# maxdoblas/QuickEd

Measured on AMD Instinct MI355X. Metric: alignments/sec + GCUPS, 10kb x 10kb 5%-error pairs, higher is better.
Workload: dtype u64; 1 GPU; banded_score, DEVICE-RESIDENT inputs: 100000 pairs/GPU x 10000 bp @ 0.05 error, bandwidth 15 %, seeded generator (SURVEY 8d), ASCII already in HBM when the clock starts, results left in HBM (end-to-end rates: e2e); pairs_per_gpu=100000, length=10000, bandwidth=15, parallelism=pairs sharded over 1 GPU(s), no data-path collective

## Files before the change

quicked_amd/csrc/qe_kernels.hip:

```cpp
#include <type_traits>
#include <hip/hip_runtime.h>
#include "qe_types.h"
#include "qe_bounded.h"
#include "qe_search.h"
#include "qe_panel.h"
#include "qe_panel_align.h"
#include "qe_pack.h"
#include "qe_tags.h"
#include "qe_check.h"

namespace qe {

#define QE_ONES (~(u64)0)
#define QE_WAVE_IN_BLOCK() ((int)(threadIdx.x >> 6))
#define QE_GROUP_INDEX() ((int)(blockIdx.x * (blockDim.x >> 6) + (threadIdx.x >> 6)))
extern __shared__ uint4 qe_dyn_lds[];

__device__ __forceinline__ u32 lo32(u64 x) { return (u32)x; }
__device__ __forceinline__ u32 hi32(u64 x) { return (u32)(x >> 32); }
__device__ __forceinline__ u64 mk64(u32 lo, u32 hi) { return ((u64)hi << 32) | lo; }

__device__ __forceinline__ int64_t tile_elem(int col, int slot, int nslots) {
    return ((int64_t)(col >> 3) * nslots + slot) * 512 + (col & 7);
}
// ... 317 lines not shown

template <int K>
__device__ __forceinline__ void run64_tall(u64 (&P)[K], u64 (&M)[K], const u64 (&a)[K], const u64 (&b)[K],
                                           u64 T0, u64 T1, u64 hinP, u64 hinM, u64& houtP, u64& houtM) {
    u32 alo[K], ahi[K], blo[K], bhi[K], Plo[K], Phi[K], Mlo[K], Mhi[K];
#pragma unroll
    for (int k = 0; k < K; ++k) {
        alo[k] = lo32(a[k]); ahi[k] = hi32(a[k]); blo[k] = lo32(b[k]); bhi[k] = hi32(b[k]);
        Plo[k] = lo32(P[k]); Phi[k] = hi32(P[k]); Mlo[k] = lo32(M[k]); Mhi[k] = hi32(M[k]);
    }
    u32 oPlo = 0, oPhi = 0, oMlo = 0, oMhi = 0;
#pragma unroll 1
    for (int half = 0; half < 2; ++half) {
        const u32 t0 = half ? hi32(T0) : lo32(T0), t1 = half ? hi32(T1) : lo32(T1);
        const u32 hp = half ? hi32(hinP) : lo32(hinP), hm = half ? hi32(hinM) : lo32(hinM);
        u32 gP = 0, gM = 0;
#pragma unroll 1
        for (int c = 0; c < 32; c += 2) {
            u32 m0[2], m1[2], cP[2], cM[2];
#pragma unroll
            for (int j = 0; j < 2; ++j) {
                m0[j] = (u32)__builtin_amdgcn_sbfe((int)t0, (u32)(c + j), 1u);
                m1[j] = (u32)__builtin_amdgcn_sbfe((int)t1, (u32)(c + j), 1u);
                cP[j] = __builtin_amdgcn_ubfe(hp, (u32)(c + j), 1u);
                cM[j] = __builtin_amdgcn_ubfe(hm, (u32)(c + j), 1u);
            }
#pragma unroll
            for (int s = 0; s <= K; ++s) {
#pragma unroll
                for (int j = 0; j < 2; ++j) {
                    const int k = s - j;
                    if (k < 0 || k >= K) continue;
                    const u32 elo = bitop3<0x90>(~(alo[k] ^ m0[j]), blo[k], m1[j]), ehi = bitop3<0x90>(~(ahi[k] ^ m0[j]), bhi[k], m1[j]);
                    if (k + 1 < K) {
                        u32 phhi, mhhi;
                        block_step_core(elo, ehi, Plo[k], Phi[k], Mlo[k], Mhi[k], cP[j], cM[j], phhi, mhhi);
                        cP[j] = phhi >> 31; cM[j] = mhhi >> 31;
                    } else {
                        block_step_collect(elo, ehi, Plo[k], Phi[k], Mlo[k], Mhi[k], cP[j], cM[j], gP, gM);
                    }
                }
            }
        }
        const u32 rP = __builtin_bitreverse32(gP), rM = __builtin_bitreverse32(gM);
        if (half) { oPhi = rP; oMhi = rM; } else { oPlo = rP; oMlo = rM; }
    }
#pragma unroll
    for (int k = 0; k < K; ++k) { P[k] = mk64(Plo[k], Phi[k]); M[k] = mk64(Mlo[k], Mhi[k]); }
    houtP = mk64(oPlo, oPhi);
    houtM = mk64(oMlo, oMhi);
}

template <int K>
__device__ __forceinline__ void slots_pass_tall(int nl, int i, int r, u64* Pv, u64* Mv, int32_t* S, const u64* pp, int p0, bool unaligned,
                                                u64 T0, u64 T1, u64& hinP, u64& hinM, u32& adv) {
    u64 P[K], M[K], a[K], b[K], a1[K], b1[K];
    int sc[K], v0[K];
    const int psh = p0 & 63;
#pragma unroll
    for (int k = 0; k < K; ++k) {
        P[k] = 0; M[k] = 0; a[k] = 0; b[k] = 0; a1[k] = 0; b1[k] = 0; sc[k] = 0;
        if (k < nl) {
            P[k] = Pv[(int64_t)(i + k) * 64]; M[k] = Mv[(int64_t)(i + k) * 64]; sc[k] = S[(int64_t)score_lds_row(r + k) * 64];
            const u64* w = pp + 3 * (int64_t)((p0 >> 6) + r + k);
            a[k] = w[0]; b[k] = w[1];
            if (unaligned) { a1[k] = w[3]; b1[k] = w[4]; }
        }
    }
    if (unaligned) {
#pragma unroll
        for (int k = 0; k < K; ++k) {
            a[k] = (a[k] >> psh) | ((a1[k] << 1) << (63 - psh));
            b[k] = (b[k] >> psh) | ((b1[k] << 1) << (63 - psh));
        }
    }
#pragma unroll
    for (int k = 0; k < K; ++k) v0[k] = __popcll(P[k]) - __popcll(M[k]);
    u64 houtP, houtM;
    run64_tall<K>(P, M, a, b, T0, T1, hinP, hinM, houtP, houtM);
    if (nl > 0) {
        int d = __popcll(houtP) - __popcll(houtM);
#pragma unroll
        for (int k = K - 1; k >= 0; --k) {
            if (k < nl) {
                S[(int64_t)score_lds_row(r + k) * 64] = sc[k] + d;
                Pv[(int64_t)(i + k - 1) * 64] = P[k]; Mv[(int64_t)(i + k - 1) * 64] = M[k];
            }
            d -= (__popcll(P[k]) - __popcll(M[k])) - v0[k];
        }
        adv += 64u * (u32)nl;
    }
    hinP = houtP; hinM = houtM;
}

__device__ __forceinline__ void run64_win2(u64& P0, u64& M0, u64& P1, u64& M1, u64 a0, u64 b0, u64 a1, u64 b1, u64 T0, u64 T1,
                                           u64 hinP, bool patch, u64 Eq_x, u64& gP, u64& gM, uint4* st, int st_stride) {
    const u32 a0lo = lo32(a0), a0hi = hi32(a0), b0lo = lo32(b0), b0hi = hi32(b0);
    const u32 a1lo = lo32(a1), a1hi = hi32(a1), b1lo = lo32(b1), b1hi = hi32(b1);
    u32 P0lo = lo32(P0), P0hi = hi32(P0), M0lo = lo32(M0), M0hi = hi32(M0);
    u32 P1lo = lo32(P1), P1hi = hi32(P1), M1lo = lo32(M1), M1hi = hi32(M1);
    u32 oPlo = 0, oPhi = 0, oMlo = 0, oMhi = 0;
#pragma unroll 1
    for (int half = 0; half < 2; ++half) {
        const u32 t0 = half ? hi32(T0) : lo32(T0), t1 = half ? hi32(T1) : lo32(T1);
        const u32 hp = half ? hi32(hinP) : lo32(hinP);
        u32 g0P = 0, g0M = 0;
        u32 m0[32], m1[32];
#pragma unroll
        for (int s = 0; s < 33; ++s) {
            if (s < 32) {
                m0[s] = (u32)__builtin_amdgcn_sbfe((int)t0, s, 1);
                m1[s] = (u32)__builtin_amdgcn_sbfe((int)t1, s, 1);
            }
            if (s >= 1) {
                const int c = s - 1;
                if ((c & 7) == 0) st[(4 * half + (c >> 3)) * st_stride] = make_uint4(P1lo, P1hi, M1lo, M1hi);
                u32 inP = g0P & 1u, inM = g0M & 1u;
                if (c == 31 && half == 1 && patch) {
                    u64 Ph, Mh, Pe = mk64(P0lo, P0hi), Me = mk64(M0lo, M0hi);
                    block_step(Eq_x, Pe, Me, 1u, 0u, Ph, Mh);
                    inP = (u32)(Ph >> 63); inM = (u32)(Mh >> 63);
                    g0P = (g0P & ~1u) | inP; g0M = (g0M & ~1u) | inM;
                }
                const u32 elo = bitop3<0x90>(~(a1lo ^ m0[c]), b1lo, m1[c]), ehi = bitop3<0x90>(~(a1hi ^ m0[c]), b1hi, m1[c]);
                u32 ph_, mh_;
                block_step_core(elo, ehi, P1lo, P1hi, M1lo, M1hi, inP, inM, ph_, mh_);
            }
            if (s < 32) {
                const u32 elo = bitop3<0x90>(~(a0lo ^ m0[s]), b0lo, m1[s]), ehi = bitop3<0x90>(~(a0hi ^ m0[s]), b0hi, m1[s]);
                block_step_fused(elo, ehi, P0lo, P0hi, M0lo, M0hi, __builtin_amdgcn_ubfe(hp, s, 1), 0u, g0P, g0M);
            }
        }
        const u32 rP = __builtin_bitreverse32(g0P), rM = __builtin_bitreverse32(g0M);
        if (half) { oPhi = rP; oMhi = rM; } else { oPlo = rP; oMlo = rM; }
    }
    P0 = mk64(P0lo, P0hi); M0 = mk64(M0lo, M0hi); P1 = mk64(P1lo, P1hi); M1 = mk64(M1lo, M1hi);
    gP = mk64(oPlo, oPhi); gM = mk64(oMlo, oMhi);
}
// ... 390 lines not shown

__global__ __launch_bounds__(256) void k_planes_iupac(IupacPlanesArgs A) {
    const int lane = threadIdx.x & 63;
    const int seq = blockIdx.x * 4 + (threadIdx.x >> 6);
    if (seq >= A.nseq) return;
    const int len = A.len[seq];
    const int nw = (len + 63) >> 6;
    const u64* __restrict__ src = A.src + A.pl_off[seq];
    u64* __restrict__ dst = A.dst + iupac_offset(A.pl_off[seq]);
    for (int r = lane; r < nw + 2; r += 64) {
        u64 o[4] = {0, 0, 0, 0};
        if (r < nw) iupac_row_from_planes3(src[3 * (int64_t)r], src[3 * (int64_t)r + 1], src[3 * (int64_t)r + 2], min(len - 64 * r, 64), A.n_empty != 0, o);
        u64* q = dst + 4 * (int64_t)r;
        q[0] = o[0]; q[1] = o[1]; q[2] = o[2]; q[3] = o[3];
    }
}

struct Geom { int cutoff, diff, prolog, ebb, fin; };
__device__ __forceinline__ Geom band_geometry(int m, int n, int cutoff_in) {
    Geom g;
    const int kend = abs(n - m) + 1;
    g.cutoff = max(max(kend, cutoff_in), 65);
    g.diff = m - n;
    const int rel = (g.cutoff - abs(g.diff) + 1) / 2;
    if (g.diff >= 0) {
        g.prolog = (rel + 63) / 64;
        g.ebb = (rel + g.diff + 63) / 64 + 1 + g.prolog;
    } else {
        g.prolog = (rel - g.diff + 63) / 64;
        g.ebb = (rel + 63) / 64 + 1 + g.prolog;
    }
    g.fin = g.prolog * 64 + g.diff;
    return g;
}

struct GroupWs {
    u64* Pv; u64* Mv; int32_t* S; int16_t* cf; int16_t* cl;
};
__device__ __forceinline__ GroupWs group_ws(uint8_t* ws, int64_t off, int ns, int nrows, int nch) {
    GroupWs w;
    uint8_t* p = ws + off;
    w.Pv = (u64*)p;              p += (int64_t)(ns + 1) * 64 * 8;
    w.Mv = (u64*)p;              p += (int64_t)(ns + 1) * 64 * 8;
    w.S = (int32_t*)p;           p += (int64_t)nrows * 64 * 4;
    w.cf = (int16_t*)p;          p += (int64_t)nch * 64 * 2;
    w.cl = (int16_t*)p;
    return w;
}

#ifndef QE_FILL_K
#define QE_FILL_K 3
#endif
constexpr bool QE_K_BANDED_LDS = true;
template <bool FILL, bool LDS = false>
__global__ __launch_bounds__(512) void k_banded(BandedArgs A) {
    static_assert(!(FILL && LDS), "the fill's state stays in the group workspace");
    const int g = QE_GROUP_INDEX(), lane = threadIdx.x & 63, t = g * 64 + lane;
    if (g * 64 >= A.T.ntasks) return;
    int pair = (t < A.T.ntasks) ? A.T.pair[t] : -1;
    if (A.only_if != nullptr && pair >= 0 && A.only_if[t] == 0) pair = -1;
    const bool have = pair >= 0;
    if (!__any(have)) return;
    int m = 1, n = 1, p0 = 0, t0 = 0, cut_in = 0, tfin = 0, prune = 0x7fffffff;
    const u64* pp = A.P.pl_p;
    const u64* tp = A.P.pl_t;
    u32 fl = 0;
    if (have) {
        m = A.T.m[t]; n = A.T.n[t]; p0 = A.T.p0[t]; t0 = A.T.t0[t];
        cut_in = A.T.cutoff[t];
        tfin = FILL ? n : A.T.tfin[t];
        if (!FILL && A.prune != nullptr) prune = A.prune[t];
        pp = A.P.pl_p + A.P.pl_p_off[pair];
        tp = A.P.pl_t + A.P.pl_t_off[pair];
        fl = A.P.flags[pair];
    }
    const bool hasN = (fl & FLAG_HAS_N) != 0;
    const Geom G = band_geometry(m, n, cut_in);
    const int thr = prune < cut_in ? prune : G.cutoff;
    const int nw = (m + 63) >> 6;
    const bool fgeom = FILL || (!LDS && A.fill_geom != 0);
    const int nsl = fgeom ? G.ebb : ((G.cutoff + 63) >> 6) + 1;
    const int stop_row = fgeom ? nw - 1 : nw;
    const int lvl_last = (m - 1) & 63;
    int first = G.prolog, last = nsl - 1, pos_v = -G.prolog, pos_h = 0;
    int max_row_init = nsl - 1;
    u32 adv = 0;

    const int gns = LDS ? A.lds_slots : A.g_nslots[g], gnr = LDS ? 0 : A.g_nrows[g], gnch = LDS ? 0 : A.g_nch[g];
    GroupWs W;
    if (LDS) {
        uint8_t* lb = (uint8_t*)qe_dyn_lds + (size_t)QE_WAVE_IN_BLOCK() * (size_t)score_lds_bytes(gns);
        W.Pv = (u64*)lb; W.Mv = W.Pv + (gns + 1) * 64; W.S = (int32_t*)(W.Mv + (gns + 1) * 64); W.cf = nullptr; W.cl = nullptr;
        if (nsl > gns) pair = -1;
    } else W = group_ws(A.ws, A.g_ws_off[g], gns, gnr, gnch);
    const bool valid = pair >= 0;
    u64* const Pv = W.Pv + 64 + lane;
    u64* const Mv = W.Mv + 64 + lane;
    int32_t* const S = W.S + lane;
    auto srow = [](int r) { return (int64_t)(LDS ? score_lds_row(r) : r) * 64; };
    uint4* const cp = FILL ? A.mat + A.g_mat_off[g] + lane : nullptr;
    const int64_t cps = (int64_t)gns * 64;
    uint4* const hw = FILL ? cp + (int64_t)QE_CPC * gnch * cps : nullptr;

    for (int s = 0; s < gns; ++s) {
        if (valid && s < nsl) {
            Pv[(int64_t)s * 64] = QE_ONES;
            Mv[(int64_t)s * 64] = 0;
            S[srow(s)] = 64 * (s + 1);
            if (FILL) cp[(int64_t)s * 64] = make_uint4(~0u, ~0u, 0u, 0u);
        }
    }
    if (FILL && valid) { W.cf[lane] = (int16_t)first; W.cl[lane] = (int16_t)last; }

    const int nfull = tfin >> 6, tail = tfin & 63;
    const int my_chunks = valid ? nfull + (tail ? 1 : 0) : 0;
    const int wave_chunks = wave_max(my_chunks);

    for (int k = 0; k < wave_chunks; ++k) {
        const int ncols = (k < nfull) ? 64 : ((k == nfull) ? tail : 0);
        const bool on = valid && ncols > 0;
        u64 T0 = 0, T1 = 0, TN = 0;
        if (on) load_planes(tp, t0 + 64 * k, T0, T1, TN);
        const int rhi = min(last, nw - 1 - pos_v);
        const int fmin = wave_min(on ? first : 0x7fffffff), fmax = wave_max(on ? first : -0x7fffffff);
        const bool rel = A.lane_rel != 0 && fmin < fmax;
        const int ib = rel ? (on ? first : 0) : 0;
        const int i0 = rel ? 0 : fmin;
        const int i1 = rel ? wave_max(on ? rhi - first : -0x7fffffff) : wave_max(on ? rhi : -0x7fffffff);
        u64 hinP = QE_ONES, hinM = 0;
        u64 qP = 0, qM = 0, qa0 = 0, qb0 = 0, qa1 = 0, qb1 = 0;
        int qS = 0, qi = -0x7fffffff;
        const int psh = p0 & 63;
        const bool unaligned = __any(psh != 0);
        auto prefetch = [&](int j) {
            const int jc = min(max(j, 0), gns - 1), rc = min(max(j + pos_v, 0), gnr - 1), rp = min(max(j + pos_v, 0), nw);
            qP = Pv[(int64_t)jc * 64]; qM = Mv[(int64_t)jc * 64]; qS = S[srow(rc)];
            const u64* w = pp + 3 * (int64_t)((p0 >> 6) + rp);
            qa0 = w[0]; qb0 = w[1];
            if (unaligned) { qa1 = w[3]; qb1 = w[4]; }
            qi = j;
        };
        if (FILL) prefetch(i0 + ib);
        for (int x = i0; x <= i1; ++x) {
            const int i = x + ib;
            const bool act = on && i >= first && i <= rhi;
            const int r = i + pos_v;
            if (!FILL) {
                const int lo = on ? first : 0x7fffffff, hi_ = on ? rhi : -0x7fffffff;
                const bool plain = !(on && (ncols != 64 || hasN));
                int nl = 0;
                auto planned = [&](int K) {
                    bool bad;
                    nl = pass_plan(i, K, lo, hi_, r, nw, plain, A.score_masked != 0, bad);
                    return !__any(bad);
                };
                if (i == first) { hinP = QE_ONES; hinM = 0; }
                const int K = __builtin_amdgcn_readfirstlane(score_pass_height(x, i0, i1, LDS && A.score_tall, planned));
                switch (K) {
                case 0: break;
                case 2: slots_pass<2, LDS>(nl, i, r, Pv, Mv, S, S, 64, pp, p0, T0, T1, hinP, hinM, adv); break;
                case 4: slots_pass<4, LDS>(nl, i, r, Pv, Mv, S, S, 64, pp, p0, T0, T1, hinP, hinM, adv); break;
                case 5: if constexpr (LDS) slots_pass_tall<5>(nl, i, r, Pv, Mv, S, pp, p0, unaligned, T0, T1, hinP, hinM, adv); break;
                case 6: if constexpr (LDS) slots_pass_tall<6>(nl, i, r, Pv, Mv, S, pp, p0, unaligned, T0, T1, hinP, hinM, adv); break;
                case 7: if constexpr (LDS) slots_pass_tall<7>(nl, i, r, Pv, Mv, S, pp, p0, unaligned, T0, T1, hinP, hinM, adv); break;
                case 8: if constexpr (LDS) slots_pass_tall<8>(nl, i, r, Pv, Mv, S, pp, p0, unaligned, T0, T1, hinP, hinM, adv); break;
                case 9: if constexpr (LDS) slots_pass_tall<9>(nl, i, r, Pv, Mv, S, pp, p0, unaligned, T0, T1, hinP, hinM, adv); break;
                default: if constexpr (LDS) slots_pass_tall<10>(nl, i, r, Pv, Mv, S, pp, p0, unaligned, T0, T1, hinP, hinM, adv); break;
                }
                if (K) { x += K - 1; continue; }
            }
            if (FILL && QE_FILL_K > 1 && A.fill_multi && x + QE_FILL_K - 1 <= i1) {
                constexpr int K = QE_FILL_K;
                bool actk[K], slowk = false;
                u32 topk[K];
#pragma unroll
                for (int q = 0; q < K; ++q) {
                    actk[q] = on && (i + q) >= first && (i + q) <= rhi;
                    topk[q] = ((i + q) == first) ? 1u : 0u;
                    slowk |= actk[q] && (ncols != 64 || hasN || (i + q + pos_v) == nw - 1);
                }
                if (!__any(slowk)) {
                    u64 P[K], M[K], a[K], b[K], oP[K], oM[K];
                    int sc[K];
#pragma unroll
                    for (int q = 0; q < K; ++q) {
                        P[q] = 0; M[q] = 0; a[q] = 0; b[q] = 0; sc[q] = 0;
                        if (actk[q]) {
                            u64 nn;
                            P[q] = Pv[(int64_t)(i + q) * 64]; M[q] = Mv[(int64_t)(i + q) * 64]; sc[q] = S[srow(r + q)];
                            load_planes(pp, p0 + 64 * (r + q), a[q], b[q], nn);
                        }
                    }
                    if (i == first) { hinP = QE_ONES; hinM = 0; }
                    uint4* const st0 = cp + (int64_t)(QE_CPC * k) * cps + (int64_t)i * 64;
                    uint4* const stl0 = cp + (int64_t)(QE_CPC * k + QE_CPC) * cps + (int64_t)(i - 1) * 64;
                    run64_skew_fill<K>(P, M, a, b, T0, T1, hinP, hinM, oP, oM, actk, topk, st0, cps,
                                       (i == 0) ? st0 + QE_CPC * cps : stl0, stl0);
#pragma unroll
                    for (int q = 0; q < K; ++q) {
                        if (actk[q]) {
                            const u64 iP = (q == 0) ? hinP : (topk[q] ? QE_ONES : oP[q > 0 ? q - 1 : 0]);
                            const u64 iM = (q == 0) ? hinM : (topk[q] ? (u64)0 : oM[q > 0 ? q - 1 : 0]);
                            hw[((int64_t)k * gns + (i + q)) * 64] = make_uint4(lo32(iP), hi32(iP), lo32(iM), hi32(iM));
                            S[srow(r + q)] = sc[q] + __popcll(oP[q]) - __popcll(oM[q]);
                            Pv[(int64_t)(i + q - 1) * 64] = P[q]; Mv[(int64_t)(i + q - 1) * 64] = M[q];
                            adv += 64u;
                        }
                    }
                    hinP = oP[K - 1]; hinM = oM[K - 1];
                    x += K - 1;
                    continue;
                }
            }
            u64 P = 0, M = 0, a = 0, b = 0, nn = 0;
            int sc = 0;
            if (FILL) {
                if (qi != i) prefetch(i);
                if (act) {
                    P = qP; M = qM; sc = qS;
                    a = (qa0 >> psh) | ((qa1 << 1) << (63 - psh));
// ... 25 lines not shown
                run64_general<FILL ? 2 : 0>(P, M, a, b, nn, T0, T1, TN, hinP, hinM, houtP, houtM, sP, sM,
                                            lastblk ? lvl_last : 63, act ? ncols : 0, true, st, cps, st_last);
            }
            if (act) {
                sc += __popcll(sP) - __popcll(sM);
                S[srow(r)] = sc;
                const int64_t dst = (ncols == 64) ? (int64_t)(i - 1) * 64 : (int64_t)i * 64;
                Pv[dst] = P;
                Mv[dst] = M;
                adv += (u32)ncols;
            }
            hinP = houtP; hinM = houtM;
        }
        if (on && ncols == 64) {
            const bool c1 = (first + 2 < last) && (G.fin > 64 * (first + 1));
            bool cut_lo = false;
            if (c1) cut_lo = S[srow(first + pos_v + 1)] + (G.fin - 64 * (first + 1)) > thr;
            if (cut_lo && pos_h >= G.prolog) first++;
            else if (!cut_lo && pos_h < G.prolog) first--;
            Pv[(int64_t)last * 64] = QE_ONES;
            Mv[(int64_t)last * 64] = 0;
            if (FILL) cp[(int64_t)(QE_CPC * k + QE_CPC) * cps + (int64_t)last * 64] = make_uint4(~0u, ~0u, 0u, 0u);
            const int pos = last + pos_v;
            S[srow(pos + 1)] = S[srow(pos)] + 64;
            max_row_init = max(max_row_init, pos + 1);
            const bool c2 = (first + 2 < last) && (64 * (last - 1) > G.fin);
            bool cut_hi = false;
            if (c2) cut_hi = S[srow(last + pos_v - 1)] + (64 * (last - 1) - G.fin) > thr;
            if (cut_hi || (pos_v + last >= stop_row)) last--;
            pos_v++;
            pos_h++;
            if (FILL) { W.cf[(int64_t)pos_h * 64 + lane] = (int16_t)first; W.cl[(int64_t)pos_h * 64 + lane] = (int16_t)last; }
        }
    }
    if (have) {
        const int row = nw - 1;
        int score = -1;
        if (valid && row <= max_row_init) {
            score = S[srow(row)];
            if (m & 63) score -= 64 - (m & 63);
        }
        A.o_score[t] = score;
        A.o_first[t] = first;
        A.o_last[t] = last;
        A.o_posv[t] = pos_v;
        A.o_maxrow[t] = max_row_init;
        A.o_adv[t] = adv;
    }
}

template __global__ void k_banded<false>(BandedArgs);
template __global__ void k_banded<true>(BandedArgs);
template __global__ void k_banded<false, true>(BandedArgs);

__global__ __launch_bounds__(256) void k_bounded_diag(BoundedArgs A) {
    const int g = QE_GROUP_INDEX(), lane = threadIdx.x & 63, t = g * 64 + lane;
    if (g * 64 >= A.T.ntasks) return;
    const int pair = (t < A.T.ntasks) ? A.T.pair[t] : -1;
    const bool valid = pair >= 0;
    if (!__any(valid)) return;
    int m = 1, n = 1, bound = 0;
    const u64* pp = A.P.pl_p;
    const u64* tp = A.P.pl_t;
    BoundedDiag S;
    S.Pv = S.Mv = S.wa = S.wb = S.wn = S.xa = S.xb = S.xn = S.force = S.track = 0; S.score = 0; S.dlo = 0;
    if (valid) {
        m = A.T.m[t]; n = A.T.n[t]; bound = A.T.cutoff[t];
        pp = A.P.pl_p + A.P.pl_p_off[pair];
        tp = A.P.pl_t + A.P.pl_t_off[pair];
        bounded_diag_init(S, pp, m, n, bound);
    }
    const int my_chunks = valid ? (n + 63) >> 6 : 0;
    const int wave_chunks = wave_max(my_chunks);
    u32 adv = 0;
    for (int k = 0; k < wave_chunks; ++k) {
        const int ncols = (k < my_chunks) ? min(64, n - 64 * k) : 0;
        const bool live = ncols > 0 && S.score <= bound;
        if (!__any(live)) break;
        if (live) {
            const u64* q = tp + 3 * (int64_t)k;
            const u64 T0 = q[0], T1 = q[1], TN = q[2];
            bounded_diag_chunk(S, pp, m, k, ncols, T0, T1, TN);
            adv += (u32)ncols;
        }
    }
    if (valid) {
        A.o_score[t] = bounded_answer(S.score, bound);
        A.o_adv[t] = adv;
    }
}

__global__ __launch_bounds__(256) void k_bounded_threshold(int nt, const int32_t* __restrict__ score, const u32* __restrict__ adv,
                                                           const int32_t* __restrict__ bound, int32_t* __restrict__ o_score, u32* __restrict__ o_adv) {
    const int t = blockIdx.x * 256 + threadIdx.x;
    if (t >= nt) return;
    o_score[t] = bounded_answer(score[t], bound[t]);
    o_adv[t] = adv[t];
}

template <int NB, class Eq = SearchEq3>
__global__ __launch_bounds__(256) void k_search(SearchArgs A) {
    const int g = QE_GROUP_INDEX(), lane = threadIdx.x & 63, t = g * 64 + lane;
    if (g * 64 >= A.T.ntasks) return;
    const int pair = (t < A.T.ntasks) ? A.T.pair[t] : -1;
    bool valid = pair >= 0;
    int m = 1, n = 0, bound = 0, in_end = 0;
// ... 3514 lines not shown
```

quicked_amd/csrc/qe_pool.h:

```cpp
#pragma once
#include <hip/hip_runtime.h>

#include <sys/syscall.h>
#include <unistd.h>

#include <algorithm>
#include <atomic>
#include <chrono>
#include <cstdio>
#include <cstdlib>
#include <cstring>
#include <memory>
#include <mutex>
#include <shared_mutex>
#include <thread>
#include <vector>

namespace qe {

struct HipError { hipError_t e; const char* what; int line; };
#define HIP_CHECK(expr)                                                             \
    do {                                                                            \
        hipError_t e__ = (expr);                                                    \
        if (e__ != hipSuccess) throw qe::HipError{e__, #expr, __LINE__};            \
    } while (0)

struct Chip {
    int cus = 256, simds = 1024;
    size_t slots2() const { return (size_t)simds * 2; }
    size_t frac2(double f) const { return (size_t)((double)simds * 2.0 * f); }
};
inline const Chip& chip(int device) {
    static Chip table[16];
    static std::once_flag once[16];
    const int d = (device >= 0 && device < 16) ? device : 0;
    std::call_once(once[d], [d] {
        int cus = 0;
        if (hipDeviceGetAttribute(&cus, hipDeviceAttributeMultiprocessorCount, d) == hipSuccess && cus > 0) { table[d].cus = cus; table[d].simds = cus * 4; }
        else (void)hipGetLastError();
    });
    return table[d];
}

enum class Sw : int {
    QuickedFast, QuickedEst, QuickedScorePass, FinishMerge, FinishMergePairs, Finishers, LaneRel, CoopG, CoopFillG, CoopLds,
    CoopTallFill, Wave, ScoreSys, Stage3Device, FormatWave, WindowedCp, WindowedQuad, WindowedSys, SplitBytes, FillSys, FillMulti,
    TraceSys, Trace, TracePool, OomWaitMs, BoundedDiag, ScoreNarrow, NarrowFit, NarrowPrune, ScoreMasked, ScoreLds, ScoreTall, TagsWave, SearchForm, SearchHitsWsKb, PanelSlices, PanelHitsRawKb, PanelAlignWsKb, Count
};
struct SwitchDef { Sw sw; const char* name; long long dflt; };
inline constexpr SwitchDef switch_defs[] = {
    {Sw::QuickedFast, "QE_QUICKED_FAST", 1},           {Sw::QuickedEst, "QE_QUICKED_EST", 0},
    {Sw::QuickedScorePass, "QE_QUICKED_SCORE_PASS", -1},
    {Sw::FinishMerge, "QE_FINISH_MERGE", 4},           {Sw::FinishMergePairs, "QE_FINISH_MERGE_PAIRS", 8192},
    {Sw::Finishers, "QE_FINISHERS", 3},                {Sw::LaneRel, "QE_LANE_REL", 1},
    {Sw::CoopG, "QE_COOP_G", 1},                       {Sw::CoopFillG, "QE_COOP_FILL_G", 1},
    {Sw::CoopLds, "QE_COOP_LDS", 1},                   {Sw::CoopTallFill, "QE_COOP_TALL_FILL", 1},
    {Sw::Wave, "QE_WAVE", -1},                         {Sw::ScoreSys, "QE_SCORE_SYS", -1},
    {Sw::Stage3Device, "QE_STAGE3_DEVICE", -1},        {Sw::FormatWave, "QE_FORMAT_WAVE", -1},
    {Sw::WindowedCp, "QE_WINDOWED_CP", 1},             {Sw::WindowedQuad, "QE_WINDOWED_QUAD", -1},
    {Sw::WindowedSys, "QE_WINDOWED_SYS", -1},          {Sw::SplitBytes, "QE_SPLIT_BYTES", 1LL << 24},
    {Sw::FillSys, "QE_FILL_SYS", -1},                  {Sw::FillMulti, "QE_FILL_MULTI", 1},
    {Sw::TraceSys, "QE_TRACE_SYS", -1},                {Sw::Trace, "QE_TRACE", 0},
    {Sw::TracePool, "QE_TRACE_POOL", 0},               {Sw::OomWaitMs, "QE_OOM_WAIT_MS", 10000},
    {Sw::BoundedDiag, "QE_BOUNDED_DIAG", -1},
    {Sw::ScoreNarrow, "QE_SCORE_NARROW", -1},
    {Sw::NarrowFit, "QE_NARROW_FIT", -1},
    {Sw::NarrowPrune, "QE_NARROW_PRUNE", -1},
    {Sw::ScoreMasked, "QE_SCORE_MASKED", 1},
    {Sw::ScoreLds, "QE_SCORE_LDS", -1},
    {Sw::ScoreTall, "QE_SCORE_TALL", -1},
    {Sw::TagsWave, "QE_TAGS_WAVE", -1},
    {Sw::SearchForm, "QE_SEARCH_FORM", -1},
    {Sw::SearchHitsWsKb, "QE_SEARCH_HITS_WS_KB", 262144},
    {Sw::PanelSlices, "QE_PANEL_SLICES", -1},
    {Sw::PanelHitsRawKb, "QE_PANEL_HITS_RAW_KB", 1048576},
    {Sw::PanelAlignWsKb, "QE_PANEL_ALIGN_WS_KB", 1048576},
};
inline constexpr int switch_count = (int)Sw::Count;
constexpr bool switch_rows_in_order() {
    for (int i = 0; i < switch_count; ++i) if ((int)switch_defs[i].sw != i) return false;
    return true;
}
static_assert(sizeof(switch_defs) / sizeof(switch_defs[0]) == (size_t)switch_count && switch_rows_in_order(), "one row per switch, in the order of Sw");

struct SwitchTable {
    bool set[switch_count];
    long long value[switch_count];
    SwitchTable() {
        for (int i = 0; i < switch_count; ++i) {
            const char* e = getenv(switch_defs[i].name);
            set[i] = e != nullptr;
            value[i] = e ? strtoll(e, nullptr, 10) : switch_defs[i].dflt;
        }
    }
};
inline std::atomic<const SwitchTable*> g_switches{nullptr};
inline const SwitchTable& switches() {
    const SwitchTable* t = g_switches.load(std::memory_order_acquire);
    if (!t) {
        const SwitchTable* fresh = new SwitchTable();
        if (g_switches.compare_exchange_strong(t, fresh, std::memory_order_acq_rel)) t = fresh;
        else delete fresh;
    }
    return *t;
}
inline void switches_reload() { g_switches.store(new SwitchTable(), std::memory_order_release); }
inline bool sw_set(Sw s) { return switches().set[(int)s]; }
inline long long sw_ll(Sw s) { return switches().value[(int)s]; }
inline int sw(Sw s) { return (int)sw_ll(s); }
inline bool pool_trace() { return sw_set(Sw::TracePool); }
inline double mono_ms() { struct timespec ts; clock_gettime(CLOCK_MONOTONIC, &ts); return ts.tv_sec * 1e3 + ts.tv_nsec * 1e-6; }

inline constexpr int QE_MAX_DEVICES = 16;
struct DeviceBook {
    std::atomic<size_t> held{0};
    std::atomic<uint64_t> epoch{0};
    std::atomic<uint64_t> pressure{0};
    std::atomic<int64_t> oom_events{0};
};
inline DeviceBook g_book[QE_MAX_DEVICES];

struct DevicePool;
struct Context;
// ... 502 lines not shown
```

quicked_amd/csrc/qe_stages.hip:

```cpp
#pragma once

namespace qe {

template <class Args> static Args with_prio(Args a) { a.prio = 1; return a; }

template <typename Kernel, typename Args>
static void launch_groups(Context& C, Kernel kernel, const Args& args, size_t ngroups, int max_waves, size_t lds_per_wave, bool chain = false,
                          size_t pin_override = 0) {
    if (ngroups == 0) return;
    const int wpb = std::min(4, max_waves);
    const unsigned blocks = (unsigned)((ngroups + wpb - 1) / wpb);
    const Chip& chp = chip(C.device);
    size_t pin = ((size_t)blocks * (size_t)std::max(1, C.in_flight) > (size_t)chp.cus) ? (size_t)54 * 1024 : (size_t)84 * 1024;
    if (chain && (size_t)blocks * (size_t)std::max(1, C.in_flight) <= (size_t)chp.cus / 2) pin = (size_t)108 * 1024;
    if (pin_override) pin = pin_override;
    const size_t lds = std::max(pin, lds_per_wave * (size_t)wpb);
    static thread_local std::vector<std::pair<const void*, int>> configured;
    const void* fn = reinterpret_cast<const void*>(kernel);
    if (std::find(configured.begin(), configured.end(), std::make_pair(fn, tl_device)) == configured.end()) {
        HIP_CHECK(hipFuncSetAttribute(fn, hipFuncAttributeMaxDynamicSharedMemorySize, 160 * 1024));
        configured.emplace_back(fn, tl_device);
    }
    hipLaunchKernelGGL(kernel, dim3(blocks), dim3(64 * wpb), lds, C.stream, args);
    HIP_CHECK(hipGetLastError());
// ... 294 lines not shown
}

static ScoreLaunch launch_banded_probe(quicked_batch& B, Context& C, const TaskList& L, bool reversed, int timed) {
    ScoreLaunch S;
    S.nt = L.pair.size();
    TaskList Ls;
    for (size_t g = 0; g < S.nt / 64; g += QE_NARROW_PROBE)
        for (size_t t = g * 64; t < g * 64 + 64; ++t) {
            const int c1 = L.pair[t] >= 0 ? narrow_cutoff(L.m[t], L.n[t], L.cutoff[t]) : 0;
            if (L.pair[t] >= 0 && c1 != L.cutoff[t]) Ls.push(L.pair[t], L.p0[t], L.m[t], L.t0[t], L.n[t], c1, L.tfin[t]);
            else Ls.push(-1, 0, 1, 0, 1, 0, 0);
        }
    BandLayout lay = band_layout(L, false, false), lays = band_layout(Ls, false, false);
    lay.mat_u4 = 0; lays.mat_u4 = 0;
    S.T = upload_tasks(L, C);
    S.D = upload_layout(lay, C);
    S.O = take_out(C, S.nt);
    ScoreLaunch P;
    P.nt = Ls.pair.size();
    P.T = upload_tasks(Ls, C);
    P.D = upload_layout(lays, C);
    P.O = take_out(C, P.nt);
    S.narrow = C.scratch_p->take<unsigned long long>(QE_NARROW_STAT);
    S.narrow_probe = true;
    HIP_CHECK(hipMemsetAsync(S.narrow, 0, QE_NARROW_STAT * sizeof(unsigned long long), C.stream));
    hipStream_t main_s = C.stream, side = C.side_stream();
    HIP_CHECK(hipEventRecord(C.ev_fork, main_s)); HIP_CHECK(hipStreamWaitEvent(side, C.ev_fork, 0));
    BandedArgs a = score_args(B, S, reversed);
    a.lane_rel = sw(Sw::LaneRel);
    TimedLaunches tl(C, timed - 1);
    launch_groups(C, k_banded<false>, a, L.ngroups(), 8, 0);
    tl.end();
    C.stream = side;
    BandedArgs b = score_args(B, P, reversed);
    b.lane_rel = a.lane_rel;
    launch_groups(C, k_banded<false>, b, Ls.ngroups(), 8, 0);
    C.stream = main_s;
    HIP_CHECK(hipEventRecord(C.ev_join, side)); HIP_CHECK(hipStreamWaitEvent(main_s, C.ev_join, 0));
    NarrowArgs x{};
    x.phase = 3; x.stride = QE_NARROW_PROBE;
    x.T = P.T.v; x.score = S.O.score; x.adv = S.O.adv; x.q_score = P.O.score; x.q_adv = P.O.adv; x.main_cutoff = S.T.cutoff; x.stat = S.narrow;
    hipLaunchKernelGGL(k_narrow, dim3((unsigned)((P.nt + 255) / 256)), dim3(256), 0, main_s, x);
    HIP_CHECK(hipGetLastError());
    return S;
}

static int score_lds_slots(const Context& C, const TaskList& L, int bound) {
    if (!QE_K_BANDED_LDS) return 0;
    const int mode = sw(Sw::ScoreLds);
    if (mode == 0 || (mode != 1 && (size_t)L.ngroups() < (size_t)chip(C.device).simds)) return 0;
    return score_lds_fits(bound) ? bound : 0;
}

static ScoreLaunch launch_banded_narrow(quicked_batch& B, Context& C, const TaskList& L, bool reversed, int timed, const BandLayout& lay, int q, int qp, int slots1) {
    ScoreLaunch S;
    S.nt = L.pair.size();
    const size_t nt = S.nt;
    S.T = upload_tasks(L, C);
    S.D = upload_layout(lay, C);
    S.O = take_out(C, nt);
    ScoreLaunch S2 = S;
    S2.O = take_out(C, nt);
    int32_t* blk = C.scratch_p->take<int32_t>(10 * nt);
    S.narrow = C.scratch_p->take<unsigned long long>(QE_NARROW_STAT);
    NarrowArgs x{};
    x.T = S.T.v; x.cut1 = blk; x.score = S.O.score; x.adv = S.O.adv;
    x.q_pair = blk + nt; x.q_p0 = blk + 2 * nt; x.q_m = blk + 3 * nt; x.q_t0 = blk + 4 * nt; x.q_n = blk + 5 * nt;
    x.q_cutoff = blk + 6 * nt; x.q_tfin = blk + 7 * nt; x.q_src = blk + 8 * nt;
    x.q_score = S2.O.score; x.q_adv = S2.O.adv; x.stat = S.narrow; x.q = q;
    x.qp = q > 0 ? qp : 0; x.prune1 = blk + 9 * nt;
    S2.T.v.pair = x.q_pair; S2.T.v.p0 = x.q_p0; S2.T.v.m = x.q_m; S2.T.v.t0 = x.q_t0; S2.T.v.n = x.q_n;
    S2.T.v.cutoff = x.q_cutoff; S2.T.v.tfin = x.q_tfin;
    const dim3 grid((unsigned)((nt + 255) / 256)), block(256);
    TimedLaunches tl(C, timed - 1);
    x.phase = 0;
    hipLaunchKernelGGL(k_narrow, grid, block, 0, C.stream, x);
    BandedArgs a = score_args(B, S, reversed);
    a.T.cutoff = x.cut1;
    if (x.qp > 0) a.prune = x.prune1;
    a.lane_rel = sw(Sw::LaneRel);
    a.lds_slots = score_lds_slots(C, L, slots1);
    a.score_tall = (a.lds_slots && sw(Sw::ScoreTall) != 0) ? 1 : 0;
    if (trace_on()) fprintf(stderr, "[qe] two-pass score: first launch of %d groups, band state in %s (%d slots), tall passes %s\n", L.ngroups(), a.lds_slots ? "LDS" : "the group workspace", a.lds_slots, a.score_tall ? "on" : "off");
    if (a.lds_slots) launch_groups(C, k_banded<false, true>, a, L.ngroups(), 8, (size_t)score_lds_bytes(a.lds_slots));
    else launch_groups(C, k_banded<false>, a, L.ngroups(), 8, 0);
    x.phase = 1;
    hipLaunchKernelGGL(k_narrow, grid, block, 0, C.stream, x);
    BandedArgs b = score_args(B, S2, reversed);
    b.lane_rel = a.lane_rel;
    launch_groups(C, k_banded<false>, b, L.ngroups(), 8, 0);
    x.phase = 2;
    hipLaunchKernelGGL(k_narrow, grid, block, 0, C.stream, x);
    HIP_CHECK(hipGetLastError());
    tl.end();
    return S;
}

static int coop_lanes(const TaskList& L, int in_flight = 1, bool fill = false) {
    const Sw force = fill ? Sw::CoopFillG : Sw::CoopG;
    const bool e = sw_set(force);
    int min_nsl = 1 << 30, n_max = 1;
    size_t live = 0;
    for (size_t t = 0; t < L.pair.size(); ++t) {
        if (L.pair[t] < 0) continue;
        ++live;
        const HGeom hg = host_geometry(L.m[t], L.n[t], L.cutoff[t]);
        min_nsl = std::min(min_nsl, fill ? hg.ebb : hg.ebb_local);
        n_max = std::max(n_max, L.n[t]);
    }
    if (live == 0) return 1;
    int G = 1;
    const Chip& chp = chip(tl_device);
    const size_t target = std::min<size_t>(2 * chp.slots2(), chp.frac2(0.34) * (size_t)std::max(1, n_max / 10000));
    if (e) G = sw(force);
    else
        while (G < 64 && ((live * G) / 64) * (size_t)std::max(1, in_flight) < target) G *= 2;
    while (G > 1 && min_nsl < 3 * G + 4) G /= 2;
    if (!e)
        while (G < 64 && min_nsl >= 2 * (2 * G) + 4 && ((live * G) / 64) * (size_t)std::max(1, in_flight) < chp.slots2() / 4) G *= 2;
    return G < 2 ? 1 : G;
}

static size_t coop_lds_bytes(int ns, int G) {
    const int NA = 64 / G, rr = ns + G + 4, cr = std::max(16, 4 * G);
    const size_t bytes = (size_t)2 * (ns + 1) * NA * 8 + (size_t)2 * rr * NA * 4 + (size_t)2 * cr * NA * 2 + (size_t)2 * NA * 4;
    return (bytes + 63) & ~(size_t)63;
}
static ScoreLaunch launch_banded_coop(quicked_batch& B, Context& C, const TaskList& L, bool reversed, int G, int timed) {
    ScoreLaunch S;
    S.nt = L.pair.size();
    const int NA = 64 / G;
    const size_t nwaves = S.nt / NA;
    std::vector<int64_t> w_off(nwaves);
    std::vector<int32_t> w_ns(nwaves), w_nr(nwaves), w_nch(nwaves);
    size_t ws_bytes = 0;
    int ns_max = 3;
// ... 1764 lines not shown
```

quicked_amd/csrc/qe_types.h:

```cpp
#pragma once
#include <stdint.h>

namespace qe {

typedef uint64_t u64;
typedef uint32_t u32;

enum : u32 { FLAG_HAS_N = 1u, FLAG_NONCANON = 2u };
enum : int { QE_CP_COLS = 16, QE_CPC = 64 / QE_CP_COLS };
enum : u32 { OP_M = 0, OP_X = 1, OP_I = 2, OP_D = 3 };

struct PairView {
    const uint8_t* asc_p;  const int64_t* asc_p_off;  const int32_t* p_len;
    const uint8_t* asc_t;  const int64_t* asc_t_off;  const int32_t* t_len;
    const u64* pl_p;  const int64_t* pl_p_off;
    const u64* pl_t;  const int64_t* pl_t_off;
    const u32* flags;
};

struct TaskView {
    int32_t ntasks;
    const int32_t* pair;
    const int32_t* p0;  const int32_t* m;
    const int32_t* t0;  const int32_t* n;
// ... 212 lines not shown
    if (s_g <= 0 || s_g >= narrow_slots(m, n, half)) return half;
    const int c = narrow_fit_cutoff(m, n, cutoff_in, s_g);
    return (c > 0 && narrow_accepts(m, n, c, cutoff_in, narrow_rhat(q, cutoff_in))) ? c : half;
}
QE_T_HD int narrow_prune(int m, int n, int cutoff_in, int c1, int qp) {
    if (qp <= 0 || c1 == cutoff_in || c1 == narrow_cutoff(m, n, cutoff_in)) return c1;
    if (narrow_slots(m, n, c1) <= 3) return c1;
    const int r = narrow_rhat(qp, cutoff_in);
    return r < c1 ? r : c1;
}
QE_T_HD bool narrow_accepts_pruned(int m, int n, int c1, int cutoff_in, int p, int r) {
    return narrow_accepts(m, n, c1, cutoff_in, r) && r <= p;
}
QE_T_HD int narrow_ratio(int m, int n, int cutoff_in, int r) {
    if (!narrow_accepts(m, n, narrow_cutoff(m, n, cutoff_in), cutoff_in, r)) return -1;
    return (int)(((long long)r * 1024 + cutoff_in - 1) / cutoff_in);
}

QE_T_HD int pass_plan(int i, int K, int lo, int hi, int r, int nw, bool plain, bool masked, bool& fallback) {
    if (!masked) {
        const bool all = i >= lo && i + K - 1 <= hi, none = i + K - 1 < lo || i > hi;
        fallback = !(all || none) || (all && (!plain || r + K - 1 >= nw - 1));
        return all ? K : 0;
    }
    const int a0 = i > lo ? i : lo, a1 = i + K - 1 < hi ? i + K - 1 : hi;
    const int nl = a1 >= a0 ? a1 - a0 + 1 : 0;
    fallback = nl > 0 && (a0 != i || !plain || r + nl - 1 >= nw - 1);
    return nl;
}
enum : int { QE_TALL_MIN = 5, QE_TALL_MAX = 10 };
QE_T_HD int tall_height(int h) {
    for (int K = QE_TALL_MAX; K >= QE_TALL_MIN; --K) {
        const int rem = h - K;
        if (rem >= 0 && rem != 3) return K;
    }
    return 0;
}
template <class Planned> QE_T_HD int score_pass_height(int x, int i0, int i1, bool tall, Planned&& planned) {
    if (tall && x == i0) {
        const int K = tall_height(i1 - i0 + 1);
        if (K && planned(K)) return K;
    }
    if (x + 3 <= i1 && planned(4)) return 4;
    if (x + 1 <= i1 && planned(2)) return 2;
    return 0;
}

QE_T_HD int score_lds_ring() { return 16; }
QE_T_HD int score_lds_cap() { return score_lds_ring() - 3; }
QE_T_HD bool score_lds_fits(int slots) { return slots >= 1 && slots <= score_lds_cap(); }
QE_T_HD int score_lds_row(int r) { return r & (score_lds_ring() - 1); }
QE_T_HD int score_lds_bytes(int slots) { return 2 * (slots + 1) * 64 * 8 + score_lds_ring() * 64 * 4; }

enum : int { QE_NARROW_STAT = 6 };
struct NarrowArgs {
    int32_t phase, stride, q;
    TaskView T;
    int32_t* cut1;
    int32_t qp = 0;  int32_t* prune1 = nullptr;
    int32_t* score;  u32* adv;
    int32_t *q_pair, *q_p0, *q_m, *q_t0, *q_n, *q_cutoff, *q_tfin, *q_src;
    const int32_t* q_score;  const u32* q_adv;
    const int32_t* main_cutoff;
    unsigned long long* stat;
};

struct BandState {
    int32_t G;
    const uint8_t* ws;  const int64_t* g_ws_off;  const int32_t* g_nslots;  const int32_t* g_nrows;  const int32_t* g_nch;
    const int32_t* first;  const int32_t* last;  const int32_t* posv;  const int32_t* maxrow;
    const int32_t* abort;
};

struct JoinArgs {
    int32_t nnodes;
    const int32_t* m;  const int32_t* n1;  const int32_t* n2;
    BandState F, R;
    BandState Ffb, Rfb;
    int32_t* o_best;  int32_t* o_score_l;  int32_t* o_score_r;  int32_t* o_ok;
};

struct SegFormatArgs {
    int32_t npairs;
    const int64_t* seg_off;
    const int32_t* seg_kind;  const int32_t* seg_a;  const int32_t* seg_b;
    const u32* runs;  const int64_t* g_runs_off;  const int32_t* nruns;
    const int32_t* g_runs_cap;  int32_t runs_by_task;
    int32_t* o_len;  int32_t* o_edits;  int32_t* o_nops;
    const int64_t* str_off;  char* pool;
    int32_t style;
};

struct SegCheckArgs {
    SegFormatArgs F;
    PairView P;
    const int32_t* root_pair;
    int32_t* o_ok;
};

struct TagStats;
struct SegTagArgs {
    SegFormatArgs F;
    PairView P;
    const int32_t* root_pair;
    int32_t want_stats, want_md;
    TagStats* o_stats;
// ... 7 lines not shown
```

Baseline: 23.62 million alignments/s.

## Build per-slot Peq match table in LDS for tall score passes

```diff
diff --git a/quicked_amd/csrc/qe_kernels.hip b/quicked_amd/csrc/qe_kernels.hip
--- a/quicked_amd/csrc/qe_kernels.hip
+++ b/quicked_amd/csrc/qe_kernels.hip
@@ -393,7 +393,85 @@
 }
 
 template <int K>
-__device__ __forceinline__ void slots_pass_tall(int nl, int i, int r, u64* Pv, u64* Mv, int32_t* S, const u64* pp, int p0, bool unaligned,
+__device__ __forceinline__ void peq_build(u64* E, const u64 (&a)[K], const u64 (&b)[K]) {
+#pragma unroll
+    for (int k = 0; k < K; ++k) {
+#pragma unroll
+        for (int sym = 0; sym < 4; ++sym) E[(sym * peq_sym_stride() + k * peq_slot_stride()) / 8] = peq_entry(a[k], b[k], sym);
+    }
+}
+template <int K, int PF>
+__device__ __forceinline__ void run64_tall_peq(u64 (&P)[K], u64 (&M)[K], const u64* E, u64 T0, u64 T1, u64 hinP, u64 hinM, u64& houtP, u64& houtM) {
+    u32 Plo[K], Phi[K], Mlo[K], Mhi[K];
+#pragma unroll
+    for (int k = 0; k < K; ++k) { Plo[k] = lo32(P[k]); Phi[k] = hi32(P[k]); Mlo[k] = lo32(M[k]); Mhi[k] = hi32(M[k]); }
+    u32 oPlo = 0, oPhi = 0, oMlo = 0, oMhi = 0;
+#pragma unroll 1
+    for (int half = 0; half < 2; ++half) {
+        const u32 t0 = half ? hi32(T0) : lo32(T0), t1 = half ? hi32(T1) : lo32(T1);
+        const u32 hp = half ? hi32(hinP) : lo32(hinP), hm = half ? hi32(hinM) : lo32(hinM);
+        u32 gP = 0, gM = 0;
+        auto read_pair = [&](u64 (&e)[2][K], int c) {
+#pragma unroll
+            for (int j = 0; j < 2; ++j) {
+                const u32 sym = __builtin_amdgcn_ubfe(t0, (u32)(c + j), 1u) + 2u * __builtin_amdgcn_ubfe(t1, (u32)(c + j), 1u);
+                const u64* row = E + sym * (u32)(peq_sym_stride() / 8);
+#pragma unroll
+                for (int k = 0; k < K; ++k) e[j][k] = row[k * (peq_slot_stride() / 8)];
+            }
+        };
+        u64 e[2][K];
+        if (PF) read_pair(e, 0);
+        constexpr int PAIRS = PF ? 2 : 1;
+#pragma unroll PAIRS
+        for (int c = 0; c < 32; c += 2) {
+            u64 nx[2][K];
+            if (PF) read_pair(nx, (c + 2) & 31);
+            else read_pair(e, c);
+            u32 cP[2], cM[2];
+#pragma unroll
+            for (int j = 0; j < 2; ++j) {
+                cP[j] = __builtin_amdgcn_ubfe(hp, (u32)(c + j), 1u);
+                cM[j] = __builtin_amdgcn_ubfe(hm, (u32)(c + j), 1u);
+            }
+#pragma unroll
+            for (int s = 0; s <= K; ++s) {
+#pragma unroll
+                for (int j = 0; j < 2; ++j) {
+                    const int k = s - j;
+                    if (k < 0 || k >= K) continue;
+                    const u32 elo = lo32(e[j][k]), ehi = hi32(e[j][k]);
+                    if (k + 1 < K) {
+                        u32 phhi, mhhi;
+                        block_step_core(elo, ehi, Plo[k], Phi[k], Mlo[k], Mhi[k], cP[j], cM[j], phhi, mhhi);
+                        cP[j] = phhi >> 31; cM[j] = mhhi >> 31;
+                    } else {
+                        block_step_collect(elo, ehi, Plo[k], Phi[k], Mlo[k], Mhi[k], cP[j], cM[j], gP, gM);
+                    }
+                }
+            }
+            if (PF) {
+#pragma unroll
+                for (int j = 0; j < 2; ++j) {
+#pragma unroll
+                    for (int k = 0; k < K; ++k) e[j][k] = nx[j][k];
+                }
+            }
+        }
+        const u32 rP = __builtin_bitreverse32(gP), rM = __builtin_bitreverse32(gM);
+        if (half) { oPhi = rP; oMhi = rM; } else { oPlo = rP; oMlo = rM; }
+    }
+#pragma unroll
+    for (int k = 0; k < K; ++k) { P[k] = mk64(Plo[k], Phi[k]); M[k] = mk64(Mlo[k], Mhi[k]); }
+    houtP = mk64(oPlo, oPhi);
+    houtM = mk64(oMlo, oMhi);
+}
+
+#ifndef QE_PEQ_PREFETCH
+#define QE_PEQ_PREFETCH 0
+#endif
+template <int K, bool RING = true, bool PEQ = false>
+__device__ __forceinline__ void slots_pass_tall(int nl, int i, int r, u64* Pv, u64* Mv, int32_t* S, u64* E, const u64* pp, int p0, bool unaligned,
                                                 u64 T0, u64 T1, u64& hinP, u64& hinM, u32& adv) {
     u64 P[K], M[K], a[K], b[K], a1[K], b1[K];
     int sc[K], v0[K];
@@ -402,7 +480,7 @@
     for (int k = 0; k < K; ++k) {
         P[k] = 0; M[k] = 0; a[k] = 0; b[k] = 0; a1[k] = 0; b1[k] = 0; sc[k] = 0;
         if (k < nl) {
-            P[k] = Pv[(int64_t)(i + k) * 64]; M[k] = Mv[(int64_t)(i + k) * 64]; sc[k] = S[(int64_t)score_lds_row(r + k) * 64];
+            P[k] = Pv[(int64_t)(i + k) * 64]; M[k] = Mv[(int64_t)(i + k) * 64]; sc[k] = S[(int64_t)(RING ? score_lds_row(r + k) : r + k) * 64];
             const u64* w = pp + 3 * (int64_t)((p0 >> 6) + r + k);
             a[k] = w[0]; b[k] = w[1];
             if (unaligned) { a1[k] = w[3]; b1[k] = w[4]; }
@@ -418,13 +496,16 @@
 #pragma unroll
     for (int k = 0; k < K; ++k) v0[k] = __popcll(P[k]) - __popcll(M[k]);
     u64 houtP, houtM;
-    run64_tall<K>(P, M, a, b, T0, T1, hinP, hinM, houtP, houtM);
+    if constexpr (PEQ) {
+        peq_build<K>(E, a, b);
+        run64_tall_peq<K, QE_PEQ_PREFETCH>(P, M, E, T0, T1, hinP, hinM, houtP, houtM);
+    } else run64_tall<K>(P, M, a, b, T0, T1, hinP, hinM, houtP, houtM);
     if (nl > 0) {
         int d = __popcll(houtP) - __popcll(houtM);
 #pragma unroll
         for (int k = K - 1; k >= 0; --k) {
             if (k < nl) {
-                S[(int64_t)score_lds_row(r + k) * 64] = sc[k] + d;
+                S[(int64_t)(RING ? score_lds_row(r + k) : r + k) * 64] = sc[k] + d;
                 Pv[(int64_t)(i + k - 1) * 64] = P[k]; Mv[(int64_t)(i + k - 1) * 64] = M[k];
             }
             d -= (__popcll(P[k]) - __popcll(M[k])) - v0[k];
@@ -921,9 +1002,11 @@
 #define QE_FILL_K 3
 #endif
 constexpr bool QE_K_BANDED_LDS = true;
-template <bool FILL, bool LDS = false>
+#define QE_K_BANDED_PEQ 1
+template <bool FILL, bool LDS = false, bool PEQ = false>
 __global__ __launch_bounds__(512) void k_banded(BandedArgs A) {
     static_assert(!(FILL && LDS), "the fill's state stays in the group workspace");
+    static_assert(!(PEQ && (FILL || LDS)), "the table form: score-only, state in the group workspace");
     const int g = QE_GROUP_INDEX(), lane = threadIdx.x & 63, t = g * 64 + lane;
     if (g * 64 >= A.T.ntasks) return;
     int pair = (t < A.T.ntasks) ? A.T.pair[t] : -1;
@@ -966,6 +1049,7 @@
     u64* const Pv = W.Pv + 64 + lane;
     u64* const Mv = W.Mv + 64 + lane;
     int32_t* const S = W.S + lane;
+    u64* const E = PEQ ? (u64*)((uint8_t*)qe_dyn_lds + (size_t)QE_WAVE_IN_BLOCK() * (size_t)peq_bytes()) + lane : nullptr;
     auto srow = [](int r) { return (int64_t)(LDS ? score_lds_row(r) : r) * 64; };
     uint4* const cp = FILL ? A.mat + A.g_mat_off[g] + lane : nullptr;
     const int64_t cps = (int64_t)gns * 64;
@@ -1024,17 +1108,17 @@
                     return !__any(bad);
                 };
                 if (i == first) { hinP = QE_ONES; hinM = 0; }
-                const int K = __builtin_amdgcn_readfirstlane(score_pass_height(x, i0, i1, LDS && A.score_tall, planned));
+                const int K = __builtin_amdgcn_readfirstlane(score_pass_height(x, i0, i1, (LDS || PEQ) && A.score_tall, planned));
                 switch (K) {
                 case 0: break;
                 case 2: slots_pass<2, LDS>(nl, i, r, Pv, Mv, S, S, 64, pp, p0, T0, T1, hinP, hinM, adv); break;
                 case 4: slots_pass<4, LDS>(nl, i, r, Pv, Mv, S, S, 64, pp, p0, T0, T1, hinP, hinM, adv); break;
-                case 5: if constexpr (LDS) slots_pass_tall<5>(nl, i, r, Pv, Mv, S, pp, p0, unaligned, T0, T1, hinP, hinM, adv); break;
-                case 6: if constexpr (LDS) slots_pass_tall<6>(nl, i, r, Pv, Mv, S, pp, p0, unaligned, T0, T1, hinP, hinM, adv); break;
-                case 7: if constexpr (LDS) slots_pass_tall<7>(nl, i, r, Pv, Mv, S, pp, p0, unaligned, T0, T1, hinP, hinM, adv); break;
-                case 8: if constexpr (LDS) slots_pass_tall<8>(nl, i, r, Pv, Mv, S, pp, p0, unaligned, T0, T1, hinP, hinM, adv); break;
-                case 9: if constexpr (LDS) slots_pass_tall<9>(nl, i, r, Pv, Mv, S, pp, p0, unaligned, T0, T1, hinP, hinM, adv); break;
-                default: if constexpr (LDS) slots_pass_tall<10>(nl, i, r, Pv, Mv, S, pp, p0, unaligned, T0, T1, hinP, hinM, adv); break;
+                case 5: if constexpr (LDS || PEQ) slots_pass_tall<5, LDS, PEQ>(nl, i, r, Pv, Mv, S, E, pp, p0, unaligned, T0, T1, hinP, hinM, adv); break;
+                case 6: if constexpr (LDS || PEQ) slots_pass_tall<6, LDS, PEQ>(nl, i, r, Pv, Mv, S, E, pp, p0, unaligned, T0, T1, hinP, hinM, adv); break;
+                case 7: if constexpr (LDS || PEQ) slots_pass_tall<7, LDS, PEQ>(nl, i, r, Pv, Mv, S, E, pp, p0, unaligned, T0, T1, hinP, hinM, adv); break;
+                case 8: if constexpr (LDS || PEQ) slots_pass_tall<8, LDS, PEQ>(nl, i, r, Pv, Mv, S, E, pp, p0, unaligned, T0, T1, hinP, hinM, adv); break;
+                case 9: if constexpr (LDS || PEQ) slots_pass_tall<9, LDS, PEQ>(nl, i, r, Pv, Mv, S, E, pp, p0, unaligned, T0, T1, hinP, hinM, adv); break;
+                default: if constexpr (LDS || PEQ) slots_pass_tall<10, LDS, PEQ>(nl, i, r, Pv, Mv, S, E, pp, p0, unaligned, T0, T1, hinP, hinM, adv); break;
                 }
                 if (K) { x += K - 1; continue; }
             }
@@ -1166,6 +1250,7 @@
 template __global__ void k_banded<false>(BandedArgs);
 template __global__ void k_banded<true>(BandedArgs);
 template __global__ void k_banded<false, true>(BandedArgs);
+template __global__ void k_banded<false, false, true>(BandedArgs);
 
 __global__ __launch_bounds__(256) void k_bounded_diag(BoundedArgs A) {
     const int g = QE_GROUP_INDEX(), lane = threadIdx.x & 63, t = g * 64 + lane;
diff --git a/quicked_amd/csrc/qe_pool.h b/quicked_amd/csrc/qe_pool.h
--- a/quicked_amd/csrc/qe_pool.h
+++ b/quicked_amd/csrc/qe_pool.h
@@ -45,7 +45,7 @@
 enum class Sw : int {
     QuickedFast, QuickedEst, QuickedScorePass, FinishMerge, FinishMergePairs, Finishers, LaneRel, CoopG, CoopFillG, CoopLds,
     CoopTallFill, Wave, ScoreSys, Stage3Device, FormatWave, WindowedCp, WindowedQuad, WindowedSys, SplitBytes, FillSys, FillMulti,
-    TraceSys, Trace, TracePool, OomWaitMs, BoundedDiag, ScoreNarrow, NarrowFit, NarrowPrune, ScoreMasked, ScoreLds, ScoreTall, TagsWave, SearchForm, SearchHitsWsKb, PanelSlices, PanelHitsRawKb, PanelAlignWsKb, Count
+    TraceSys, Trace, TracePool, OomWaitMs, BoundedDiag, ScoreNarrow, NarrowFit, NarrowPrune, ScoreMasked, ScoreLds, ScoreTall, ScorePeq, TagsWave, SearchForm, SearchHitsWsKb, PanelSlices, PanelHitsRawKb, PanelAlignWsKb, Count
 };
 struct SwitchDef { Sw sw; const char* name; long long dflt; };
 inline constexpr SwitchDef switch_defs[] = {
@@ -69,6 +69,7 @@
     {Sw::ScoreMasked, "QE_SCORE_MASKED", 1},
     {Sw::ScoreLds, "QE_SCORE_LDS", -1},
     {Sw::ScoreTall, "QE_SCORE_TALL", -1},
+    {Sw::ScorePeq, "QE_SCORE_PEQ", -1},
     {Sw::TagsWave, "QE_TAGS_WAVE", -1},
     {Sw::SearchForm, "QE_SEARCH_FORM", -1},
     {Sw::SearchHitsWsKb, "QE_SEARCH_HITS_WS_KB", 262144},
diff --git a/quicked_amd/csrc/qe_stages.hip b/quicked_amd/csrc/qe_stages.hip
--- a/quicked_amd/csrc/qe_stages.hip
+++ b/quicked_amd/csrc/qe_stages.hip
@@ -370,6 +370,27 @@
     return score_lds_fits(bound) ? bound : 0;
 }
 
+static bool score_peq(const Context& C, const TaskList& L, bool tall_lds) {
+    (void)C; (void)L;
+#ifdef QE_K_BANDED_PEQ
+    if (!QE_K_BANDED_LDS) return false;
+    const int mode = sw(Sw::ScorePeq);
+    if (mode == 0 || sw(Sw::ScoreLds) == 1 || sw(Sw::ScoreTall) == 0) return false;
+    if (mode != 1 && !tall_lds) return false;
+    static thread_local std::vector<std::pair<int, int>> per_cu;
+    for (const auto& d : per_cu) if (d.first == tl_device) return d.second >= 2;
+    const void* fn = reinterpret_cast<const void*>(k_banded<false, false, true>);
+    int nb = 0;
+    HIP_CHECK(hipFuncSetAttribute(fn, hipFuncAttributeMaxDynamicSharedMemorySize, 160 * 1024));
+    if (hipOccupancyMaxActiveBlocksPerMultiprocessor(&nb, fn, 256, (size_t)4 * (size_t)peq_bytes()) != hipSuccess) { (void)hipGetLastError(); nb = 0; }
+    if (trace_on()) fprintf(stderr, "[qe] table form: %d workgroups of %d B of LDS per CU\n", nb, 4 * peq_bytes());
+    per_cu.emplace_back(tl_device, nb);
+    return nb >= 2;
+#else
+    return false;
+#endif
+}
+
 static ScoreLaunch launch_banded_narrow(quicked_batch& B, Context& C, const TaskList& L, bool reversed, int timed, const BandLayout& lay, int q, int qp, int slots1) {
     ScoreLaunch S;
     S.nt = L.pair.size();
@@ -399,7 +420,13 @@
     a.lane_rel = sw(Sw::LaneRel);
     a.lds_slots = score_lds_slots(C, L, slots1);
     a.score_tall = (a.lds_slots && sw(Sw::ScoreTall) != 0) ? 1 : 0;
-    if (trace_on()) fprintf(stderr, "[qe] two-pass score: first launch of %d groups, band state in %s (%d slots), tall passes %s\n", L.ngroups(), a.lds_slots ? "LDS" : "the group workspace", a.lds_slots, a.score_tall ? "on" : "off");
+    const bool peq = score_peq(C, L, a.lds_slots != 0 && a.score_tall != 0);
+    if (peq) { a.lds_slots = 0; a.score_tall = 1; }
+    if (trace_on()) fprintf(stderr, "[qe] two-pass score: first launch of %d groups, band state in %s (%d slots), tall passes %s%s\n", L.ngroups(), a.lds_slots ? "LDS" : "the group workspace", a.lds_slots, a.score_tall ? "on" : "off", peq ? ", Eq from a table in LDS" : "");
+#ifdef QE_K_BANDED_PEQ
+    if (peq) launch_groups(C, k_banded<false, false, true>, a, L.ngroups(), 8, (size_t)peq_bytes());
+    else
+#endif
     if (a.lds_slots) launch_groups(C, k_banded<false, true>, a, L.ngroups(), 8, (size_t)score_lds_bytes(a.lds_slots));
     else launch_groups(C, k_banded<false>, a, L.ngroups(), 8, 0);
     x.phase = 1;
diff --git a/quicked_amd/csrc/qe_types.h b/quicked_amd/csrc/qe_types.h
--- a/quicked_amd/csrc/qe_types.h
+++ b/quicked_amd/csrc/qe_types.h
@@ -288,6 +288,13 @@
 QE_T_HD int score_lds_row(int r) { return r & (score_lds_ring() - 1); }
 QE_T_HD int score_lds_bytes(int slots) { return 2 * (slots + 1) * 64 * 8 + score_lds_ring() * 64 * 4; }
 
+QE_T_HD int peq_cap() { return QE_TALL_MAX; }
+QE_T_HD int peq_slot_stride() { return 64 * 8; }
+QE_T_HD int peq_sym_stride() { return peq_cap() * peq_slot_stride(); }
+QE_T_HD int peq_bytes() { return 4 * peq_sym_stride(); }
+QE_T_HD int peq_offset(int sym, int slot, int lane) { return sym * peq_sym_stride() + slot * peq_slot_stride() + lane * 8; }
+QE_T_HD u64 peq_entry(u64 a, u64 b, int sym) { return ((sym & 1) ? a : ~a) & ((sym & 2) ? b : ~b); }
+
 enum : int { QE_NARROW_STAT = 6 };
 struct NarrowArgs {
     int32_t phase, stride, q;
```

Result: faster. 24.85 million alignments/s (median of 6 runs) (+5.2%).
